# sdwyc/ROLO

Measured on AMD Instinct MI355X. Metric: scans/sec (128k-pt frame, 20 GN iters), higher is better.
Workload: dtype f64

## Files before the change

### rolo_amd/csrc/knn_cov.hip

```cpp
#include <cstdio>
#include <cstring>
#include <string.h>
#include "rolo_internal.hpp"
#include "switches.hpp"
#include "dev_math.hpp"
#include "voxel_dev.hpp"
#ifdef ROLO_KNN_ROCPRIM_SORT
#include <rocprim/rocprim.hpp>
#endif
#include <cfloat>
#include <climits>

namespace rolo {

namespace {


constexpr int BBOX_BLOCKS = 128;
constexpr int BBOX_PART = 16;

__global__ __launch_bounds__(256) void bbox_kernel(KnnPair A, int* bbox) {
  __shared__ float smn[4][3], smx[4][3];
  const int which = blockIdx.x / BBOX_BLOCKS, blk = blockIdx.x - which * BBOX_BLOCKS;
  const float4* __restrict__ p = A.c[which].xyz;
  const int n = A.c[which].n;
  float mn[3] = {FLT_MAX, FLT_MAX, FLT_MAX}, mx[3] = {-FLT_MAX, -FLT_MAX, -FLT_MAX};
  for (int i = blk * blockDim.x + threadIdx.x; i < n; i += BBOX_BLOCKS * blockDim.x) {
    float4 q = p[i];
    mn[0] = fminf(mn[0], q.x); mn[1] = fminf(mn[1], q.y); mn[2] = fminf(mn[2], q.z);
    mx[0] = fmaxf(mx[0], q.x); mx[1] = fmaxf(mx[1], q.y); mx[2] = fmaxf(mx[2], q.z);
  }
#pragma unroll
  for (int d = 0; d < 3; d++) {
#pragma unroll
    for (int off = 32; off > 0; off >>= 1) {
      mn[d] = fminf(mn[d], __shfl_xor(mn[d], off, 64));
      mx[d] = fmaxf(mx[d], __shfl_xor(mx[d], off, 64));
    }
  }
  const int wv = threadIdx.x >> 6;
  if ((threadIdx.x & 63) == 0) {
#pragma unroll
    for (int d = 0; d < 3; d++) { smn[wv][d] = mn[d]; smx[wv][d] = mx[d]; }
  }
  __syncthreads();
  if (threadIdx.x < 3) {
    const int d = threadIdx.x;
    const float a = fminf(fminf(smn[0][d], smn[1][d]), fminf(smn[2][d], smn[3][d]));
    const float b = fmaxf(fmaxf(smx[0][d], smx[1][d]), fmaxf(smx[2][d], smx[3][d]));
    int* part = bbox + BBOX_PART + (which * BBOX_BLOCKS + blk) * 6;
    part[d] = f2ord(a);
    part[3 + d] = f2ord(b);
  }
}

ROLO_DEV uint32_t expand10(uint32_t v) {
  v &= 0x3ffu;
  v = (v | (v << 16)) & 0x030000ffu;
  v = (v | (v << 8)) & 0x0300f00fu;
  v = (v | (v << 4)) & 0x030c30c3u;
  v = (v | (v << 2)) & 0x09249249u;
  return v;
}

ROLO_DEV uint32_t hilbert30(uint32_t x, uint32_t y, uint32_t z) {
  uint32_t X[3] = {x, y, z};
  for (uint32_t Q = 512; Q > 1; Q >>= 1) {
    const uint32_t P = Q - 1;
#pragma unroll
    for (int i = 0; i < 3; i++) {
      if (X[i] & Q) X[0] ^= P;
      else { const uint32_t t = (X[0] ^ X[i]) & P; X[0] ^= t; X[i] ^= t; }
    }
  }
  X[1] ^= X[0]; X[2] ^= X[1];
  uint32_t t = 0;
  for (uint32_t Q = 512; Q > 1; Q >>= 1) if (X[2] & Q) t ^= Q - 1;
  X[0] ^= t; X[1] ^= t; X[2] ^= t;
  return (expand10(X[0]) << 2) | (expand10(X[1]) << 1) | expand10(X[2]);
}

#ifndef ROLO_SORT_NB
#define ROLO_SORT_NB 128
#endif
#ifndef ROLO_SORT_T
#define ROLO_SORT_T 1024
#endif
#ifndef ROLO_SORT_EPT
#define ROLO_SORT_EPT 2
#endif
#ifndef ROLO_SORT_BITS
#define ROLO_SORT_BITS 9
#endif
#ifndef ROLO_SORT_PASSES
#define ROLO_SORT_PASSES 3
#endif
constexpr int SORT_BITS = ROLO_SORT_BITS, SORT_PASSES = ROLO_SORT_PASSES, SORT_D = 1 << SORT_BITS, KEY_BITS = SORT_BITS * SORT_PASSES;
static_assert(KEY_BITS >= 25 && KEY_BITS <= 31, "curve index + cloud bit");
constexpr int SORT_NB = ROLO_SORT_NB, SORT_T = ROLO_SORT_T;
static_assert(SORT_T % SORT_D == 0 || SORT_D % SORT_T == 0, "threads share the count prologue by digit");
static_assert(SORT_T >= 12 * 64, "the key kernel folds the 12 box components with one wavefront each");
ROLO_DEV int sort_tile(int n_total) { return ((n_total + SORT_NB - 1) / SORT_NB + SORT_T - 1) / SORT_T * SORT_T; }

constexpr int SORT_EPT = ROLO_SORT_EPT;
__global__ __launch_bounds__(SORT_T) void sort_scatter_kernel(const uint32_t* __restrict__ kin, const uint32_t* __restrict__ vin, uint32_t* __restrict__ kout,
                                                             uint32_t* __restrict__ vout, int n, int tile, int pass, int* __restrict__ cnt ,
                                                             VoxelFuse vf) {
  ROLO_ALL_KERNEL_PRIO();
  if ((int)blockIdx.x >= SORT_NB) {
    const int nt = vf.n_tgt, quarter = (nt + SORT_PASSES - 1) / SORT_PASSES;
    const int i = pass * quarter + ((int)blockIdx.x - SORT_NB) * SORT_T + (int)threadIdx.x;
    voxel_insert_point(vf.tab, vf.tgt_xyz, i < (pass + 1) * quarter ? nt : 0, i, vf.tgt_keys, vf.tgt_slot, vf.counters);
    return;
  }
  __shared__ int wcnt[SORT_T / 64][SORT_D];
  __shared__ int base[SORT_D], run[SORT_D], wsum[SORT_D / 64];
  const int tid = threadIdx.x, lane = tid & 63, wv = tid >> 6, blk = blockIdx.x;
  const int* __restrict__ c = cnt + (size_t)pass * SORT_NB * SORT_D;
  for (int k = tid; k < (SORT_T / 64) * SORT_D; k += SORT_T) (&wcnt[0][0])[k] = 0;
  constexpr int Q = SORT_T / SORT_D;
  static_assert(Q >= 1, "at least one thread per digit");
  __shared__ int part[2][Q][SORT_D];
  {
    const int d = tid & (SORT_D - 1), q = tid / SORT_D;
    int tot = 0, bef = 0;
#pragma unroll 16
    for (int b = q; b < SORT_NB; b += Q) { const int v = c[b * SORT_D + d]; tot += v; bef += b < blk ? v : 0; }
    part[0][q][d] = tot; part[1][q][d] = bef;
  }
  __syncthreads();
  int t = 0;
  if (tid < SORT_D) {
    int before = 0;
#pragma unroll
    for (int q = 0; q < Q; q++) { t += part[0][q][tid]; before += part[1][q][tid]; }
    run[tid] = before;
    int incl = t;
#pragma unroll
    for (int off = 1; off < 64; off <<= 1) { const int o = __shfl_up(incl, off, 64); if (lane >= off) incl += o; }
    if (lane == 63) wsum[wv] = incl;
    t = incl - t;
  }
  __syncthreads();
  if (tid < SORT_D) { int add = 0; for (int w = 0; w < wv; w++) add += wsum[w]; base[tid] = t + add; }
  __syncthreads();
  const int shift = SORT_BITS * pass;
  for (int r0 = 0; r0 < tile; r0 += SORT_T * SORT_EPT) {
    uint32_t key[SORT_EPT]; int off[SORT_EPT], e[SORT_EPT];
#pragma unroll
    for (int j = 0; j < SORT_EPT; j++) {
      e[j] = blk * tile + r0 + (wv * SORT_EPT + j) * 64 + lane;
      const bool valid = e[j] < n && (r0 + (wv * SORT_EPT + j) * 64 + lane) < tile;
      key[j] = valid ? kin[e[j]] : 0u;
      if (!valid) e[j] = -1;
    }
#pragma unroll
    for (int j = 0; j < SORT_EPT; j++) {
      const bool valid = e[j] >= 0;
      const int d = (int)((key[j] >> shift) & (uint32_t)(SORT_D - 1));
      unsigned long long m = __ballot(valid);
#pragma unroll
      for (int bit = 0; bit < SORT_BITS; bit++) {
        const bool one = (d >> bit) & 1;
        const unsigned long long bl = __ballot(one);
        m &= one ? bl : ~bl;
      }
      const int rank = __popcll(m & ((1ull << lane) - 1ull));
      int old = 0;
      if (valid && rank == 0) { old = wcnt[wv][d]; wcnt[wv][d] = old + __popcll(m); }
      const int leader = valid ? __ffsll((long long)m) - 1 : lane;
      old = __shfl(old, leader, 64);
      off[j] = old + rank;
    }
    __syncthreads();
    if (tid < SORT_D) {
      int acc = run[tid];
#pragma unroll
      for (int w = 0; w < SORT_T / 64; w++) { const int v = wcnt[w][tid]; wcnt[w][tid] = acc; acc += v; }
      run[tid] = acc;
    }
    __syncthreads();
#pragma unroll
    for (int j = 0; j < SORT_EPT; j++) {
      if (e[j] >= 0) {
        const int d = (int)((key[j] >> shift) & (uint32_t)(SORT_D - 1));
        const int dest = base[d] + wcnt[wv][d] + off[j];
        kout[dest] = key[j]; vout[dest] = vin[e[j]];
      }
    }
    if (r0 + SORT_T * SORT_EPT < tile) {
      __syncthreads();
      for (int k = tid; k < (SORT_T / 64) * SORT_D; k += SORT_T) (&wcnt[0][0])[k] = 0;
      __syncthreads();
    }
  }
}

constexpr int VF_CLEAR_BLOCKS = 64;
__global__ __launch_bounds__(SORT_T) void morton_kernel(KnnPair A, int* __restrict__ bbox, uint32_t* __restrict__ keys, uint32_t* __restrict__ vals, int n_total, int tile,
                                                       int* __restrict__ cnt, VoxelFuse vf) {
  ROLO_ALL_KERNEL_PRIO();
  if ((int)blockIdx.x >= SORT_NB) {
    const size_t n_words = 2 * ((size_t)vf.tab.mask + 1);
    for (size_t k = (size_t)((int)blockIdx.x - SORT_NB) * SORT_T + threadIdx.x; k < n_words; k += (size_t)VF_CLEAR_BLOCKS * SORT_T) vf.tab.keys[k] = KEY_EMPTY;
    if (blockIdx.x == SORT_NB && threadIdx.x < 3) vf.counters[threadIdx.x] = 0;
    return;
  }
  __shared__ int hist[SORT_D];
  __shared__ float par[2][4];
  const int tid = threadIdx.x, blk = blockIdx.x;
  if (tid < SORT_D) hist[tid] = 0;
  __shared__ int fin[12];
  {
    const int w = tid >> 6, lane = tid & 63;
    if (w < 6 * A.n_clouds) {
      const bool is_min = (w % 6) < 3;
      int v = is_min ? INT_MAX : INT_MIN;
      const int* __restrict__ bp = A.c[w / 6].bpart; const int nbp = A.c[w / 6].n_bpart;
      for (int b = lane; b < nbp; b += 64) { const int o = bp[b * 6 + (w % 6)]; v = is_min ? min(v, o) : max(v, o); }
#pragma unroll
      for (int off = 32; off > 0; off >>= 1) { const int o = __shfl_xor(v, off, 64); v = is_min ? min(v, o) : max(v, o); }
      if (lane == 0) { fin[w] = v; if (blk == 0) bbox[w] = v; }
    }
  }
  __syncthreads();
  if (vf.enabled && blk == 0 && tid == 0) {
    float m = 0.f;
    for (int k = 0; k < 6; k++) { const int o = fin[6 * vf.which + k]; m = fmaxf(m, fabsf(__int_as_float(o >= 0 ? o : o ^ 0x7fffffff))); }
    vf.counters[3] = __float_as_int(m);
  }
  if (tid < A.n_clouds) {
    const int* bb = fin + 6 * tid;
    const float mnx = ord2f(bb[0]), mny = ord2f(bb[1]), mnz = ord2f(bb[2]);
    const float ext = fmaxf(fmaxf(ord2f(bb[3]) - mnx, ord2f(bb[4]) - mny), ord2f(bb[5]) - mnz);
    par[tid][0] = mnx; par[tid][1] = mny; par[tid][2] = mnz; par[tid][3] = ext > 0.f ? 1024.0f / ext : 0.f;
  }
  __syncthreads();
  const int n0 = A.c[0].n;
  for (int r = tid; r < tile; r += SORT_T) {
    const int e = blk * tile + r;
    if (e >= n_total) break;
    const int which = e >= n0 ? 1 : 0;
    const int i = e - (which ? n0 : 0);
    const float4 q = A.c[which].xyz[i];
    const float mnx = par[which][0], mny = par[which][1], mnz = par[which][2], sc = par[which][3];
    const int ix = min(1023, max(0, (int)((q.x - mnx) * sc)));
    const int iy = min(1023, max(0, (int)((q.y - mny) * sc)));
    const int iz = min(1023, max(0, (int)((q.z - mnz) * sc)));
#ifndef ROLO_KNN_MORTON
    const uint32_t key = (hilbert30((uint32_t)ix, (uint32_t)iy, (uint32_t)iz) >> (31 - KEY_BITS)) | ((uint32_t)which << (KEY_BITS - 1));
#else
    const uint32_t key = ((expand10(ix) | (expand10(iy) << 1) | (expand10(iz) << 2)) >> (31 - KEY_BITS)) | ((uint32_t)which << (KEY_BITS - 1));
#endif
    keys[e] = key;
    vals[e] = (uint32_t)i;
    atomicAdd(&hist[key & (uint32_t)(SORT_D - 1)], 1);
  }
  __syncthreads();
  if (cnt && tid < SORT_D) cnt[blk * SORT_D + tid] = hist[tid];
}

__global__ __launch_bounds__(SORT_T) void sort_hist_kernel(const uint32_t* __restrict__ keys, int n, int tile, int pass, int* __restrict__ cnt) {
  ROLO_ALL_KERNEL_PRIO();
  __shared__ int hist[SORT_D];
  const int tid = threadIdx.x, blk = blockIdx.x;
  if (tid < SORT_D) hist[tid] = 0;
  __syncthreads();
  const int shift = SORT_BITS * pass;
  for (int r = tid; r < tile; r += SORT_T) {
    const int e = blk * tile + r;
    if (e >= n) break;
    atomicAdd(&hist[(keys[e] >> shift) & (uint32_t)(SORT_D - 1)], 1);
  }
  __syncthreads();
  if (tid < SORT_D) cnt[(size_t)pass * SORT_NB * SORT_D + blk * SORT_D + tid] = hist[tid];
}

__global__ __launch_bounds__(256) void leaf_kernel(KnnPair A, int split, const uint32_t* __restrict__ order) {
  ROLO_ALL_KERNEL_PRIO();
  const int which = (int)blockIdx.x >= split ? 1 : 0;
  const float4* __restrict__ p = A.c[which].xyz;
  const int n = A.c[which].n, n_leaves = A.c[which].n_leaves, P = A.c[which].P;
  float4* sorted = A.c[which].sorted; float4* boxes = A.c[which].boxes;
  order += which ? A.c[0].n : 0;
  const int s = ((int)blockIdx.x - (which ? split : 0)) * blockDim.x + threadIdx.x;
  const int g = s / KNN_LEAF;
  float4 o = make_float4(INFINITY, INFINITY, INFINITY, __int_as_float(INT_MAX));
  if (g < P && s < n) {
    const uint32_t idx = order[s];
    const float4 q = p[idx];
    o = make_float4(q.x, q.y, q.z, __int_as_float((int)idx));
  }
  if (g >= P) return;
  const bool real = __float_as_int(o.w) != INT_MAX;
  float lox = real ? o.x : INFINITY, loy = real ? o.y : INFINITY, loz = real ? o.z : INFINITY;
  float hix = real ? o.x : -INFINITY, hiy = real ? o.y : -INFINITY, hiz = real ? o.z : -INFINITY;
  if (g < n_leaves) sorted[s] = o;
#pragma unroll
  for (int m = 1; m < KNN_LEAF; m <<= 1) {
    lox = fminf(lox, __shfl_xor(lox, m)); loy = fminf(loy, __shfl_xor(loy, m)); loz = fminf(loz, __shfl_xor(loz, m));
    hix = fmaxf(hix, __shfl_xor(hix, m)); hiy = fmaxf(hiy, __shfl_xor(hiy, m)); hiz = fmaxf(hiz, __shfl_xor(hiz, m));
  }
  if ((s & (KNN_LEAF - 1)) == 0) {
    boxes[2 * (size_t)(P + g)] = make_float4(lox, loy, loz, 0.f);
    boxes[2 * (size_t)(P + g) + 1] = make_float4(hix, hiy, hiz, 0.f);
  }
  constexpr int LPB = 256 / KNN_LEAF;
  if (P >= LPB) {
    __shared__ float4 nlo[LPB], nhi[LPB];
    const int lt = threadIdx.x / KNN_LEAF;
    if ((s & (KNN_LEAF - 1)) == 0) { nlo[lt] = make_float4(lox, loy, loz, 0.f); nhi[lt] = make_float4(hix, hiy, hiz, 0.f); }
    __syncthreads();
    const size_t g0 = (size_t)P + (size_t)(g - lt);
    int m = LPB; size_t first = g0;
    while (m > 1) {
      const int half = m >> 1;
      first >>= 1;
      float4 a, b;
      const int u = threadIdx.x;
      if (u < half) {
        const float4 l0 = nlo[2 * u], l1 = nlo[2 * u + 1], h0 = nhi[2 * u], h1 = nhi[2 * u + 1];
        a = make_float4(fminf(l0.x, l1.x), fminf(l0.y, l1.y), fminf(l0.z, l1.z), 0.f);
        b = make_float4(fmaxf(h0.x, h1.x), fmaxf(h0.y, h1.y), fmaxf(h0.z, h1.z), 0.f);
      }
      __syncthreads();
      if (u < half) { nlo[u] = a; nhi[u] = b; boxes[2 * (first + u)] = a; boxes[2 * (first + u) + 1] = b; }
      __syncthreads();
      m = half;
    }
  }
}

__global__ __launch_bounds__(256) void tree_reduce_kernel(float4* boxes0, int count_in0, int chunk0, int split, float4* boxes1, int count_in1, int chunk1) {
  ROLO_ALL_KERNEL_PRIO();
  __shared__ float4 lo[512], hi[512];
  const bool second = (int)blockIdx.x >= split;
  float4* boxes = second ? boxes1 : boxes0;
  const int count_in = second ? count_in1 : count_in0, chunk = second ? chunk1 : chunk0;
  const int b = (int)blockIdx.x - (second ? split : 0), t = threadIdx.x;
  const size_t base_in = (size_t)count_in + (size_t)b * chunk;
  for (int i = t; i < chunk; i += 256) { lo[i] = boxes[2 * (base_in + i)]; hi[i] = boxes[2 * (base_in + i) + 1]; }
  __syncthreads();
  int m = chunk, level_count = count_in;
  while (m > 1) {
    const int half = m >> 1;
    level_count >>= 1;
    float4 nlo, nhi;
    if (t < half) {
      float4 a = lo[2 * t], c = lo[2 * t + 1], e = hi[2 * t], f = hi[2 * t + 1];
      nlo = make_float4(fminf(a.x, c.x), fminf(a.y, c.y), fminf(a.z, c.z), 0.f);
      nhi = make_float4(fmaxf(e.x, f.x), fmaxf(e.y, f.y), fmaxf(e.z, f.z), 0.f);
    }
    __syncthreads();
    if (t < half) {
      lo[t] = nlo; hi[t] = nhi;
      size_t h = (size_t)level_count + (size_t)b * half + t;
      boxes[2 * h] = nlo; boxes[2 * h + 1] = nhi;
    }
    __syncthreads();
    m = half;
  }
}

struct Rot2 { double c, s; };

ROLO_DEV void make_jacobi(double x, double y, double z, Rot2& r) {
  double deno = 2.0 * fabs(y);
  if (deno < DBL_MIN) { r.c = 1; r.s = 0; return; }
  double tau = (x - z) / deno;
  double w = sqrt(tau * tau + 1.0);
  double t = 1.0 / ((tau > 0) ? tau + w : tau - w);
  double n = 1.0 / sqrt(t * t + 1.0);
  const double mag = fabs(t) * n + fabs(y) * 0.0;
  const int flip = ((t > 0) ? (int)0x80000000 : 0) ^ (__double2hiint(y) & (int)0x80000000);
  r.s = __hiloint2double(__double2hiint(mag) ^ flip, __double2loint(mag));
  r.c = n;
}

template <int P_, int Q_>
ROLO_DEV bool jacobi_pair(double (&W)[9], double (&U)[9], double (&V)[9], double& max_diag) {
  const double threshold = fmax(DBL_MIN, 2.0 * DBL_EPSILON * max_diag);
  if (!(fabs(W[P_ * 3 + Q_]) > threshold || fabs(W[Q_ * 3 + P_]) > threshold)) return false;
  double m00 = W[P_ * 3 + P_], m01 = W[P_ * 3 + Q_], m10 = W[Q_ * 3 + P_], m11 = W[Q_ * 3 + Q_];
  Rot2 rot1;
  double t = m00 + m11, d = m10 - m01;
  if (fabs(d) < DBL_MIN) { rot1.s = 0; rot1.c = 1; }
  else {
    double u = t / d; double tmp = sqrt(1.0 + u * u);
    if (fabs(u) >= 0x1p-500 && tmp <= 0x1p499) { const double rt = div_den(tmp); rot1.s = div_shared(1.0, tmp, rt); rot1.c = div_shared(u, tmp, rt); }
    else { rot1.s = 1.0 / tmp; rot1.c = u / tmp; }
  }
  double n00 = rot1.c * m00 + rot1.s * m10, n01 = rot1.c * m01 + rot1.s * m11, n11 = -rot1.s * m01 + rot1.c * m11;
  Rot2 jr; make_jacobi(n00, n01, n11, jr);
  Rot2 jl; { double c2 = jr.c, s2 = -jr.s; jl.c = rot1.c * c2 - rot1.s * s2; jl.s = rot1.c * s2 + rot1.s * c2; }
#pragma unroll
  for (int k = 0; k < 3; k++) { double x = W[P_ * 3 + k], y = W[Q_ * 3 + k]; W[P_ * 3 + k] = jl.c * x + jl.s * y; W[Q_ * 3 + k] = -jl.s * x + jl.c * y; }
#pragma unroll
  for (int k = 0; k < 3; k++) { double x = U[k * 3 + P_], y = U[k * 3 + Q_]; U[k * 3 + P_] = jl.c * x + jl.s * y; U[k * 3 + Q_] = -jl.s * x + jl.c * y; }
#pragma unroll
  for (int k = 0; k < 3; k++) { double x = W[k * 3 + P_], y = W[k * 3 + Q_]; W[k * 3 + P_] = jr.c * x - jr.s * y; W[k * 3 + Q_] = jr.s * x + jr.c * y; }
#pragma unroll
  for (int k = 0; k < 3; k++) { double x = V[k * 3 + P_], y = V[k * 3 + Q_]; V[k * 3 + P_] = jr.c * x - jr.s * y; V[k * 3 + Q_] = jr.s * x + jr.c * y; }
  max_diag = fmax(max_diag, fmax(fabs(W[P_ * 3 + P_]), fabs(W[Q_ * 3 + Q_])));
  return true;
}

ROLO_DEV void swap_cols(double (&M)[9], int a, int b) {
#pragma unroll
  for (int k = 0; k < 3; k++) { double t = M[k * 3 + a]; M[k * 3 + a] = M[k * 3 + b]; M[k * 3 + b] = t; }
}

ROLO_DEV void jacobi_svd3(const double (&A)[9], double (&U)[9], double (&sv)[3], double (&V)[9]) {
  double scale = 0;
#pragma unroll
  for (int i = 0; i < 9; i++) scale = fmax(scale, fabs(A[i]));
  if (!(scale > 0) || !isfinite(scale)) scale = 1.0;
  double W[9];
#pragma unroll
  for (int i = 0; i < 9; i++) { W[i] = A[i] / scale; U[i] = (i % 4 == 0) ? 1.0 : 0.0; V[i] = (i % 4 == 0) ? 1.0 : 0.0; }
  double max_diag = fmax(fabs(W[0]), fmax(fabs(W[4]), fabs(W[8])));
  for (int sweep = 0; sweep < 100; sweep++) {
    bool any = false;
    any |= jacobi_pair<1, 0>(W, U, V, max_diag);
    any |= jacobi_pair<2, 0>(W, U, V, max_diag);
    any |= jacobi_pair<2, 1>(W, U, V, max_diag);
    if (!any) break;
  }
#pragma unroll
  for (int i = 0; i < 3; i++) {
    double a = fabs(W[i * 4]);
    sv[i] = a * scale;
    if (a != 0) { double sgn = copysign(1.0, W[i * 4]) + W[i * 4] * 0.0; U[0 * 3 + i] *= sgn; U[1 * 3 + i] *= sgn; U[2 * 3 + i] *= sgn; }
  }
  if (sv[1] > sv[0] && sv[1] >= sv[2]) { double t = sv[0]; sv[0] = sv[1]; sv[1] = t; swap_cols(U, 0, 1); swap_cols(V, 0, 1); }
  else if (sv[2] > sv[0] && sv[2] > sv[1]) { double t = sv[0]; sv[0] = sv[2]; sv[2] = t; swap_cols(U, 0, 2); swap_cols(V, 0, 2); }
  if (sv[2] > sv[1]) { double t = sv[1]; sv[1] = sv[2]; sv[2] = t; swap_cols(U, 1, 2); swap_cols(V, 1, 2); }
}

ROLO_DEV void inv3(const double (&A)[9], double (&o)[9]) {
  double c00 = A[4] * A[8] - A[5] * A[7], c01 = A[2] * A[7] - A[1] * A[8], c02 = A[1] * A[5] - A[2] * A[4];
  double c10 = A[5] * A[6] - A[3] * A[8], c11 = A[0] * A[8] - A[2] * A[6], c12 = A[2] * A[3] - A[0] * A[5];
  double c20 = A[3] * A[7] - A[4] * A[6], c21 = A[1] * A[6] - A[0] * A[7], c22 = A[0] * A[4] - A[1] * A[3];
  double det = A[0] * c00 + A[1] * c10 + A[2] * c20;
  double inv = 1.0 / det;
  o[0] = c00 * inv; o[1] = c01 * inv; o[2] = c02 * inv; o[3] = c10 * inv; o[4] = c11 * inv; o[5] = c12 * inv; o[6] = c20 * inv; o[7] = c21 * inv; o[8] = c22 * inv;
}

ROLO_DEV void knn_covariance_finish(double cxx, double cxy, double cxz, double cyy, double cyz, double czz, int n, int qi, int reg,
                                    double* __restrict__ cov, double (&c6)[6], double* __restrict__ nrm = nullptr) {
  double out[9];
  double U[9], V[9];

  if (reg == ROLO_REG_NONE) {
    out[0] = cxx; out[1] = cxy; out[2] = cxz; out[3] = cxy; out[4] = cyy; out[5] = cyz; out[6] = cxz; out[7] = cyz; out[8] = czz;
  } else if (reg == ROLO_REG_FROBENIUS) {
    double C[9] = {cxx + 1e-3, cxy, cxz, cxy, cyy + 1e-3, cyz, cxz, cyz, czz + 1e-3};
    double Ci[9]; inv3(C, Ci);
    double nrm = 0;
#pragma unroll
    for (int i = 0; i < 9; i++) nrm += Ci[i] * Ci[i];
    nrm = sqrt(nrm);
#pragma unroll
    for (int i = 0; i < 9; i++) Ci[i] /= nrm;
    inv3(Ci, out);
  } else {
    const double A[9] = {cxx, cxy, cxz, cxy, cyy, cyz, cxz, cyz, czz};
    double sv[3];
    jacobi_svd3(A, U, sv, V);
    double v0 = 1, v1 = 1, v2 = 1e-3;
    if (reg == ROLO_REG_MIN_EIG) { v0 = fmax(sv[0], 1e-3); v1 = fmax(sv[1], 1e-3); v2 = fmax(sv[2], 1e-3); }
    else if (reg == ROLO_REG_NORMALIZED_MIN_EIG) {
      const double m = fmax(sv[0], fmax(sv[1], sv[2])), q0 = sv[0] / m, q1 = sv[1] / m, q2 = sv[2] / m;
      v0 = q0 < 1e-3 ? 1e-3 : q0; v1 = q1 < 1e-3 ? 1e-3 : q1; v2 = q2 < 1e-3 ? 1e-3 : q2;
    }
    else if (reg == ROLO_REG_PLANE_S) { double s = sv[0] + sv[1] + sv[2]; v0 = sv[0] / s; v1 = sv[1] / s; v2 = 1e-3; }
#pragma unroll
    for (int a = 0; a < 3; a++)
#pragma unroll
      for (int b = 0; b < 3; b++) out[a * 3 + b] = (U[a * 3 + 0] * v0) * V[b * 3 + 0] + (U[a * 3 + 1] * v1) * V[b * 3 + 1] + (U[a * 3 + 2] * v2) * V[b * 3 + 2];
  }
  const size_t pitch = (size_t)n;
  c6[0] = out[0]; c6[1] = 0.5 * (out[1] + out[3]); c6[2] = 0.5 * (out[2] + out[6]); c6[3] = out[4]; c6[4] = 0.5 * (out[5] + out[7]); c6[5] = out[8];
  if (reg == ROLO_REG_PLANE) {
    const double s3 = U[0 * 3 + 2] * V[0 * 3 + 2] + U[1 * 3 + 2] * V[1 * 3 + 2] + U[2 * 3 + 2] * V[2 * 3 + 2];
    const double al = sqrt(1.0 - (s3 < 0 ? -1e-3 : 1e-3));
    const double mx = al * V[0 * 3 + 2], my = al * V[1 * 3 + 2], mz = al * V[2 * 3 + 2];
    const double s1 = U[0 * 3 + 0] * V[0 * 3 + 0] + U[1 * 3 + 0] * V[1 * 3 + 0] + U[2 * 3 + 0] * V[2 * 3 + 0];
    const double s2 = U[0 * 3 + 1] * V[0 * 3 + 1] + U[1 * 3 + 1] * V[1 * 3 + 1] + U[2 * 3 + 1] * V[2 * 3 + 1];
    const bool plane_form = s1 > 0 && s2 > 0;
    if (plane_form) {
      const double p6[6] = {1.0 - mx * mx, -(mx * my), -(mx * mz), 1.0 - my * my, -(my * mz), 1.0 - mz * mz};
      double dev = 0;
#pragma unroll
      for (int d = 0; d < 6; d++) dev = fmax(dev, fabs(c6[d] - p6[d]));
      if (!(dev <= 0x1p-46)) {
#pragma unroll
        for (int d = 0; d < 6; d++) c6[d] = p6[d];
      }
    }
    if (nrm) { nrm[qi] = plane_form ? mx : __builtin_nan(""); nrm[pitch + qi] = my; nrm[2 * pitch + qi] = mz; }
  }
#pragma unroll
  for (int d = 0; d < 6; d++) cov[d * pitch + qi] = c6[d];
}

template <int KMAX>
ROLO_DEV void knn_neighbourhood_moments(const int (&ki)[KMAX], int kk, const float4* __restrict__ orig, double (&m6)[6]) {
  float px[KMAX], py[KMAX], pz[KMAX];
#pragma unroll
  for (int u = 0; u < KMAX; u++) {
    const float4 p = (u < kk) ? orig[ki[u]] : make_float4(0.f, 0.f, 0.f, 0.f);
    px[u] = p.x; py[u] = p.y; pz[u] = p.z;
  }
  double mx = 0, my = 0, mz = 0;
#pragma unroll
  for (int u = 0; u < KMAX; u++) if (u < kk) { mx += (double)px[u]; my += (double)py[u]; mz += (double)pz[u]; }
  mx /= kk; my /= kk; mz /= kk;
  double cxx = 0, cxy = 0, cxz = 0, cyy = 0, cyz = 0, czz = 0;
#pragma unroll
  for (int u = 0; u < KMAX; u++) if (u < kk) {
    const double ax = (double)px[u] - mx, ay = (double)py[u] - my, az = (double)pz[u] - mz;
    cxx += ax * ax; cxy += ax * ay; cxz += ax * az; cyy += ay * ay; cyz += ay * az; czz += az * az;
  }
  m6[0] = cxx / kk; m6[1] = cxy / kk; m6[2] = cxz / kk; m6[3] = cyy / kk; m6[4] = cyz / kk; m6[5] = czz / kk;
}

template <int KMAX>
ROLO_DEV void knn_covariance_tail(const int (&ki)[KMAX], int kk, const float4* __restrict__ orig, int n, int qi, int reg,
                                  double* __restrict__ cov, double (&c6)[6], double* __restrict__ nrm = nullptr) {
  double m6[6];
  knn_neighbourhood_moments<KMAX>(ki, kk, orig, m6);
  knn_covariance_finish(m6[0], m6[1], m6[2], m6[3], m6[4], m6[5], n, qi, reg, cov, c6, nrm);
}

ROLO_DEV void knn_covariance_tail_loop(const int32_t* __restrict__ nbr, size_t n_sorted, int j, int kk, const float4* __restrict__ orig, int n, int qi, int reg,
                                       double* __restrict__ cov, double (&c6)[6], double* __restrict__ nrm = nullptr) {
  double mx = 0, my = 0, mz = 0;
  for (int u = 0; u < kk; u++) { const float4 p = orig[nbr[(size_t)u * n_sorted + j]]; mx += (double)p.x; my += (double)p.y; mz += (double)p.z; }
  mx /= kk; my /= kk; mz /= kk;
  double cxx = 0, cxy = 0, cxz = 0, cyy = 0, cyz = 0, czz = 0;
  for (int u = 0; u < kk; u++) {
    const float4 p = orig[nbr[(size_t)u * n_sorted + j]];
    const double ax = (double)p.x - mx, ay = (double)p.y - my, az = (double)p.z - mz;
    cxx += ax * ax; cxy += ax * ay; cxz += ax * az; cyy += ay * ay; cyz += ay * az; czz += az * az;
  }
  cxx /= kk; cxy /= kk; cxz /= kk; cyy /= kk; cyz /= kk; czz /= kk;
  knn_covariance_finish(cxx, cxy, cxz, cyy, cyz, czz, n, qi, reg, cov, c6, nrm);
}
}
}

#include "knn_walk.hpp"

namespace rolo {

bool knn_voxel_fuse_supported() {
#ifdef ROLO_KNN_ROCPRIM_SORT
  return false;
#else
  return true;
#endif
}

size_t knn_bbox_ints() { return BBOX_PART + 2 * BBOX_BLOCKS * 6; }

size_t knn_sort_temp_bytes(int n) {
#ifdef ROLO_KNN_ROCPRIM_SORT
  size_t bytes = 0;
  (void)rocprim::radix_sort_pairs(nullptr, bytes, (uint32_t*)nullptr, (uint32_t*)nullptr, (uint32_t*)nullptr, (uint32_t*)nullptr,
                                  (size_t)n, 0, 31, (hipStream_t)0);
  return bytes;
#else
  (void)n;
  return sizeof(int) * SORT_PASSES * SORT_NB * SORT_D;
#endif
}

hipError_t launch_knn_build(const KnnPair& A_in, void* sort_tmp, size_t sort_tmp_bytes, uint32_t* keys0, uint32_t* keys1,
                            uint32_t* vals0, uint32_t* vals1, int* bbox, const VoxelFuse& vf, hipStream_t s) {
  KnnPair A = A_in;
  bool have_parts = true;
  for (int i = 0; i < A.n_clouds; i++) have_parts = have_parts && A.c[i].bpart != nullptr && A.c[i].n_bpart > 0;
  if (!have_parts) for (int i = 0; i < A.n_clouds; i++) { A.c[i].bpart = bbox + BBOX_PART + i * BBOX_BLOCKS * 6; A.c[i].n_bpart = BBOX_BLOCKS; }
  const int nc = A.n_clouds;
  const int n_total = A.c[0].n + (nc > 1 ? A.c[1].n : 0);
#ifdef ROLO_KNN_ROCPRIM_SORT
  const int tile_ = ((n_total + SORT_NB - 1) / SORT_NB + SORT_T - 1) / SORT_T * SORT_T;
  if (!have_parts) bbox_kernel<<<BBOX_BLOCKS * nc, 256, 0, s>>>(A, bbox);
  morton_kernel<<<SORT_NB + (vf.enabled ? VF_CLEAR_BLOCKS : 0), SORT_T, 0, s>>>(A, bbox, keys0, vals0, n_total, tile_, nullptr, vf);
  hipError_t e = rocprim::radix_sort_pairs(sort_tmp, sort_tmp_bytes, keys0, keys1, vals0, vals1, (size_t)n_total, 0, nc > 1 ? KEY_BITS : KEY_BITS - 1, s);
  if (e != hipSuccess) return e;
  const uint32_t* order = vals1;
#else
  (void)sort_tmp_bytes;
  int* cnt = static_cast<int*>(sort_tmp);
  const int gvf = vf.enabled ? ((vf.n_tgt + SORT_PASSES - 1) / SORT_PASSES + SORT_T - 1) / SORT_T : 0;
  const int tile = ((n_total + SORT_NB - 1) / SORT_NB + SORT_T - 1) / SORT_T * SORT_T;
  if (!have_parts) bbox_kernel<<<BBOX_BLOCKS * nc, 256, 0, s>>>(A, bbox);
  morton_kernel<<<SORT_NB + (vf.enabled ? VF_CLEAR_BLOCKS : 0), SORT_T, 0, s>>>(A, bbox, keys0, vals0, n_total, tile, cnt, vf);
  uint32_t *ki = keys0, *vi = vals0, *ko = keys1, *vo = vals1;
  for (int p = 0; p < SORT_PASSES; p++) {
    if (p > 0) sort_hist_kernel<<<SORT_NB, SORT_T, 0, s>>>(ki, n_total, tile, p, cnt);
    sort_scatter_kernel<<<SORT_NB + gvf, SORT_T, 0, s>>>(ki, vi, ko, vo, n_total, tile, p, cnt, vf);
    uint32_t* t1 = ki; ki = ko; ko = t1; t1 = vi; vi = vo; vo = t1;
  }
  const uint32_t* order = vi;
#endif
  static_assert(256 % KNN_LEAF == 0 && (KNN_LEAF & (KNN_LEAF - 1)) == 0, "leaf_kernel reduces a leaf inside a wavefront");
  const int l0 = (A.c[0].P * KNN_LEAF + 255) / 256, l1 = nc > 1 ? (A.c[1].P * KNN_LEAF + 255) / 256 : 0;
  leaf_kernel<<<l0 + l1, 256, 0, s>>>(A, l0, order);
  constexpr int LPB = 256 / KNN_LEAF;
  int count0 = A.c[0].P >= LPB ? A.c[0].P / LPB : A.c[0].P, count1 = nc > 1 ? (A.c[1].P >= LPB ? A.c[1].P / LPB : A.c[1].P) : 1;
  while (count0 > 1 || count1 > 1) {
    const int chunk0 = count0 < 512 ? count0 : 512, chunk1 = count1 < 512 ? count1 : 512;
    const int b0 = count0 > 1 ? count0 / chunk0 : 0, b1 = count1 > 1 ? count1 / chunk1 : 0;
    tree_reduce_kernel<<<b0 + b1, 256, 0, s>>>(A.c[0].boxes, count0, chunk0, b0, nc > 1 ? A.c[1].boxes : nullptr, count1, chunk1);
    if (count0 > 1) count0 /= chunk0;
    if (count1 > 1) count1 /= chunk1;
  }
  return hipGetLastError();
}

#ifdef ROLO_KNN_STATS
extern "C" int rolo_debug_wave_records(unsigned* out ) {
  (void)hipDeviceSynchronize();
  return hipMemcpyFromSymbol(out, HIP_SYMBOL(g_knn_wave_rec), sizeof(unsigned) * 16384 * 8) == hipSuccess ? 0 : -1;
}
#endif

static inline int slice_blocks(const KnnCloud& c) { return (c.q_end - c.q_begin + 255) / 256; }

constexpr int KNN_SUB_MAX_PACKETS = 1792;
hipError_t launch_knn_walk(const KnnPair& A, int k, hipStream_t s, int* lanes_out, bool device_busy, bool moments) {
  if (lanes_out) *lanes_out = 1;
  constexpr int QPB = 256;
  const int n0 = A.c[0].q_end - A.c[0].q_begin, n1 = A.n_clouds > 1 ? A.c[1].q_end - A.c[1].q_begin : 0;
  const int g0 = (n0 + QPB - 1) / QPB, g1 = (n1 + QPB - 1) / QPB;
  if (g0 + g1 == 0) return hipSuccess;
  for (int i = 0; i < A.n_clouds; i++) if (A.c[i].q_end > A.c[i].q_begin && A.c[i].q_begin % 64 != 0) return hipErrorInvalidValue;
  for (int i = 0; i < A.n_clouds; i++) if (A.c[i].n >= KNN_MAX_POINTS) return hipErrorInvalidValue;
  if (k > 64) {
    KnnPair R = A;
    for (int r = 0; 64 * r < k; r++) {
      const int kr = k - 64 * r < 64 ? k - 64 * r : 64;
      for (int i = 0; i < R.n_clouds; i++) { R.c[i].slot0 = 64 * r; R.c[i].k_total = k; }
      if (r == 0) knn_walk_kernel<64><<<g0 + g1, 256, 0, s>>>(R, g0, kr);
      else knn_walk_kernel<64, true><<<g0 + g1, 256, 0, s>>>(R, g0, kr);
    }
    return hipGetLastError();
  }
  if (k == 20) {
    const int sub_env = switches().knn_sub;
    const int packets = (n0 + 63) / 64 + (n1 + 63) / 64;
    const int lanes = sub_env < 0 ? (packets <= KNN_SUB_MAX_PACKETS ? 4 : (device_busy ? 0 : 2)) : (sub_env == 2 ? 2 : (sub_env ? 4 : 0));
    if (lanes_out) *lanes_out = lanes ? lanes : 1;
    if (lanes == 4) { const int s0 = (n0 + 63) / 64, s1 = (n1 + 63) / 64; if (moments) knn_walk_sub_kernel<4, true><<<s0 + s1, 256, 0, s>>>(A, s0); else knn_walk_sub_kernel<4><<<s0 + s1, 256, 0, s>>>(A, s0); }
    else if (lanes == 2) { const int s0 = (n0 + 127) / 128, s1 = (n1 + 127) / 128; if (moments) knn_walk_sub_kernel<2, true><<<s0 + s1, 256, 0, s>>>(A, s0); else knn_walk_sub_kernel<2><<<s0 + s1, 256, 0, s>>>(A, s0); }
    else if (moments) knn_walk_kernel<20, false, true><<<g0 + g1, 256, 0, s>>>(A, g0, k);
    else knn_walk_kernel<20><<<g0 + g1, 256, 0, s>>>(A, g0, k);
  }
  else if (k > 32) knn_walk_kernel<64><<<g0 + g1, 256, 0, s>>>(A, g0, k);
  else knn_walk_kernel<32><<<g0 + g1, 256, 0, s>>>(A, g0, k);
  return hipGetLastError();
}

hipError_t launch_knn_unstage(const KnnPair& A, bool own_slice_only, const VoxelFuse& vf, hipStream_t s) {
  const int g0 = own_slice_only ? slice_blocks(A.c[0]) : (A.c[0].n_sorted + 255) / 256;
  const int g1 = A.n_clouds > 1 ? (own_slice_only ? slice_blocks(A.c[1]) : (A.c[1].n_sorted + 255) / 256) : 0;
  if (g0 + g1 == 0) return hipSuccess;
  VoxelFuse v = vf;
  if (own_slice_only) v.enabled = 0;
  knn_unstage_kernel<<<g0 + g1, 256, 0, s>>>(A, g0, own_slice_only ? 1 : 0, v);
  return hipGetLastError();
}

hipError_t launch_knn_tail(const KnnPair& A, int k, int regularization, const VoxelFuse& vf, hipStream_t s, bool moments) {
  const int g0 = slice_blocks(A.c[0]), g1 = A.n_clouds > 1 ? slice_blocks(A.c[1]) : 0;
  if (g0 + g1 == 0) return hipSuccess;
  if (k > 64) knn_tail_loop_kernel<<<g0 + g1, 256, 0, s>>>(A, g0, k, regularization, vf);
  else if (k == 20 && moments) knn_tail_kernel<20, true><<<g0 + g1, 256, 0, s>>>(A, g0, k, regularization, vf);
  else if (k == 20) knn_tail_kernel<20><<<g0 + g1, 256, 0, s>>>(A, g0, k, regularization, vf);
  else if (k <= 32) knn_tail_kernel<32><<<g0 + g1, 256, 0, s>>>(A, g0, k, regularization, vf);
  else knn_tail_kernel<64><<<g0 + g1, 256, 0, s>>>(A, g0, k, regularization, vf);
  return hipGetLastError();
}

}
```

Baseline: 5217.

## Sort each cloud separately in radix sort, dropping cloud bit and vals pre-write

The radix sort now gives each cloud its own half of the workgroups and its own segment of the key buffer. Keys no longer carry a cloud bit, so the curve index keeps a full 27 bits over the three passes. The key kernel stops writing a vals array, because the first scatter pass derives the value from the element index. The per-digit count prologue only sums rows for the block's own cloud, in unrolled chunks. It also removes the rocprim path. The changes trim memory traffic and prologue work but add per-block geometry arithmetic.

```diff
diff --git a/rolo_amd/csrc/knn_cov.hip b/rolo_amd/csrc/knn_cov.hip
--- a/rolo_amd/csrc/knn_cov.hip
+++ b/rolo_amd/csrc/knn_cov.hip
@@ -5,9 +5,7 @@
 #include "switches.hpp"
 #include "dev_math.hpp"
 #include "voxel_dev.hpp"
-#ifdef ROLO_KNN_ROCPRIM_SORT
-#include <rocprim/rocprim.hpp>
-#endif
+#include "sort_tiles.hpp"
 #include <cfloat>
 #include <climits>
 
@@ -80,12 +78,6 @@
   return (expand10(X[0]) << 2) | (expand10(X[1]) << 1) | expand10(X[2]);
 }
 
-#ifndef ROLO_SORT_NB
-#define ROLO_SORT_NB 128
-#endif
-#ifndef ROLO_SORT_T
-#define ROLO_SORT_T 1024
-#endif
 #ifndef ROLO_SORT_EPT
 #define ROLO_SORT_EPT 2
 #endif
@@ -96,16 +88,14 @@
 #define ROLO_SORT_PASSES 3
 #endif
 constexpr int SORT_BITS = ROLO_SORT_BITS, SORT_PASSES = ROLO_SORT_PASSES, SORT_D = 1 << SORT_BITS, KEY_BITS = SORT_BITS * SORT_PASSES;
-static_assert(KEY_BITS >= 25 && KEY_BITS <= 31, "curve index + cloud bit");
-constexpr int SORT_NB = ROLO_SORT_NB, SORT_T = ROLO_SORT_T;
-static_assert(SORT_T % SORT_D == 0 || SORT_D % SORT_T == 0, "threads share the count prologue by digit");
-static_assert(SORT_T >= 12 * 64, "the key kernel folds the 12 box components with one wavefront each");
-ROLO_DEV int sort_tile(int n_total) { return ((n_total + SORT_NB - 1) / SORT_NB + SORT_T - 1) / SORT_T * SORT_T; }
+static_assert(KEY_BITS >= 1 && KEY_BITS <= 30, "the leading bits of the 30-bit curve index");
+static_assert(SORT_T % SORT_D == 0, "threads share the count prologue by digit");
+static_assert(SORT_T >= 6 * 64, "the key kernel folds the 6 box components of its cloud with one wavefront each");
 
 constexpr int SORT_EPT = ROLO_SORT_EPT;
 __global__ __launch_bounds__(SORT_T) void sort_scatter_kernel(const uint32_t* __restrict__ kin, const uint32_t* __restrict__ vin, uint32_t* __restrict__ kout,
-                                                             uint32_t* __restrict__ vout, int n, int tile, int pass, int* __restrict__ cnt ,
-                                                             VoxelFuse vf) {
+                                                             uint32_t* __restrict__ vout, int n0, int n1, int n_clouds, int pass,
+                                                             int* __restrict__ cnt , VoxelFuse vf) {
   ROLO_ALL_KERNEL_PRIO();
   if ((int)blockIdx.x >= SORT_NB) {
     const int nt = vf.n_tgt, quarter = (nt + SORT_PASSES - 1) / SORT_PASSES;
@@ -115,18 +105,34 @@
   }
   __shared__ int wcnt[SORT_T / 64][SORT_D];
   __shared__ int base[SORT_D], run[SORT_D], wsum[SORT_D / 64];
-  const int tid = threadIdx.x, lane = tid & 63, wv = tid >> 6, blk = blockIdx.x;
-  const int* __restrict__ c = cnt + (size_t)pass * SORT_NB * SORT_D;
+  const int tid = threadIdx.x, lane = tid & 63, wv = tid >> 6;
+  const SortGeom g = sort_geom((int)blockIdx.x, n0, n1, n_clouds);
+  const int* __restrict__ c = cnt + ((size_t)pass * SORT_NB + g.row0) * SORT_D;
   for (int k = tid; k < (SORT_T / 64) * SORT_D; k += SORT_T) (&wcnt[0][0])[k] = 0;
-  constexpr int Q = SORT_T / SORT_D;
+  constexpr int Q = SORT_T / SORT_D, CH = 16;
   static_assert(Q >= 1, "at least one thread per digit");
+  static_assert((SORT_NB / 2) % (Q * CH) == 0, "whole chunks of rows per thread, for a pair's cloud and for a lone one");
   __shared__ int part[2][Q][SORT_D];
   {
     const int d = tid & (SORT_D - 1), q = tid / SORT_D;
-    int tot = 0, bef = 0;
-#pragma unroll 16
-    for (int b = q; b < SORT_NB; b += Q) { const int v = c[b * SORT_D + d]; tot += v; bef += b < blk ? v : 0; }
-    part[0][q][d] = tot; part[1][q][d] = bef;
+    const int nbef = g.tile > q ? (g.tile - q + Q - 1) / Q : 0;
+    int bef = 0, aft = 0;
+    for (int i0 = 0; i0 < g.tiles / Q; i0 += CH) {
+      int v[CH];
+#pragma unroll
+      for (int i = 0; i < CH; i++) v[i] = c[(q + (i0 + i) * Q) * SORT_D + d];
+      if (i0 + CH <= nbef) {
+#pragma unroll
+        for (int i = 0; i < CH; i++) bef += v[i];
+      } else if (i0 >= nbef) {
+#pragma unroll
+        for (int i = 0; i < CH; i++) aft += v[i];
+      } else {
+#pragma unroll
+        for (int i = 0; i < CH; i++) { if (i0 + i < nbef) bef += v[i]; else aft += v[i]; }
+      }
+    }
+    part[0][q][d] = bef + aft; part[1][q][d] = bef;
   }
   __syncthreads();
   int t = 0;
@@ -145,12 +151,14 @@
   if (tid < SORT_D) { int add = 0; for (int w = 0; w < wv; w++) add += wsum[w]; base[tid] = t + add; }
   __syncthreads();
   const int shift = SORT_BITS * pass;
-  for (int r0 = 0; r0 < tile; r0 += SORT_T * SORT_EPT) {
+  kin += g.offset; kout += g.offset; vout += g.offset;
+  if (pass > 0) vin += g.offset;
+  for (int r0 = 0; r0 < g.len; r0 += SORT_T * SORT_EPT) {
     uint32_t key[SORT_EPT]; int off[SORT_EPT], e[SORT_EPT];
 #pragma unroll
     for (int j = 0; j < SORT_EPT; j++) {
-      e[j] = blk * tile + r0 + (wv * SORT_EPT + j) * 64 + lane;
-      const bool valid = e[j] < n && (r0 + (wv * SORT_EPT + j) * 64 + lane) < tile;
+      e[j] = g.first + r0 + (wv * SORT_EPT + j) * 64 + lane;
+      const bool valid = e[j] < g.last;
       key[j] = valid ? kin[e[j]] : 0u;
       if (!valid) e[j] = -1;
     }
@@ -185,10 +193,10 @@
       if (e[j] >= 0) {
         const int d = (int)((key[j] >> shift) & (uint32_t)(SORT_D - 1));
         const int dest = base[d] + wcnt[wv][d] + off[j];
-        kout[dest] = key[j]; vout[dest] = vin[e[j]];
+        kout[dest] = key[j]; vout[dest] = pass > 0 ? vin[e[j]] : (uint32_t)e[j];
       }
     }
-    if (r0 + SORT_T * SORT_EPT < tile) {
+    if (r0 + SORT_T * SORT_EPT < g.len) {
       __syncthreads();
       for (int k = tid; k < (SORT_T / 64) * SORT_D; k += SORT_T) (&wcnt[0][0])[k] = 0;
       __syncthreads();
@@ -197,8 +205,7 @@
 }
 
 constexpr int VF_CLEAR_BLOCKS = 64;
-__global__ __launch_bounds__(SORT_T) void morton_kernel(KnnPair A, int* __restrict__ bbox, uint32_t* __restrict__ keys, uint32_t* __restrict__ vals, int n_total, int tile,
-                                                       int* __restrict__ cnt, VoxelFuse vf) {
+__global__ __launch_bounds__(SORT_T) void morton_kernel(KnnPair A, int* __restrict__ bbox, uint32_t* __restrict__ keys, int* __restrict__ cnt, VoxelFuse vf) {
   ROLO_ALL_KERNEL_PRIO();
   if ((int)blockIdx.x >= SORT_NB) {
     const size_t n_words = 2 * ((size_t)vf.tab.mask + 1);
@@ -207,71 +214,66 @@
     return;
   }
   __shared__ int hist[SORT_D];
-  __shared__ float par[2][4];
+  __shared__ float par[4];
   const int tid = threadIdx.x, blk = blockIdx.x;
+  const SortGeom g = sort_geom(blk, A.c[0].n, A.c[1].n, A.n_clouds);
+  const KnnCloud& C = A.c[g.cloud];
   if (tid < SORT_D) hist[tid] = 0;
-  __shared__ int fin[12];
+  __shared__ int fin[6];
   {
     const int w = tid >> 6, lane = tid & 63;
-    if (w < 6 * A.n_clouds) {
-      const bool is_min = (w % 6) < 3;
+    if (w < 6) {
+      const bool is_min = w < 3;
       int v = is_min ? INT_MAX : INT_MIN;
-      const int* __restrict__ bp = A.c[w / 6].bpart; const int nbp = A.c[w / 6].n_bpart;
-      for (int b = lane; b < nbp; b += 64) { const int o = bp[b * 6 + (w % 6)]; v = is_min ? min(v, o) : max(v, o); }
+      const int* __restrict__ bp = C.bpart; const int nbp = C.n_bpart;
+      for (int b = lane; b < nbp; b += 64) { const int o = bp[b * 6 + w]; v = is_min ? min(v, o) : max(v, o); }
 #pragma unroll
       for (int off = 32; off > 0; off >>= 1) { const int o = __shfl_xor(v, off, 64); v = is_min ? min(v, o) : max(v, o); }
-      if (lane == 0) { fin[w] = v; if (blk == 0) bbox[w] = v; }
-    }
-  }
-  __syncthreads();
-  if (vf.enabled && blk == 0 && tid == 0) {
+      if (lane == 0) { fin[w] = v; if (g.tile == 0) bbox[6 * g.cloud + w] = v; }
+    }
+  }
+  __syncthreads();
+  if (vf.enabled && g.cloud == vf.which && g.tile == 0 && tid == 0) {
     float m = 0.f;
-    for (int k = 0; k < 6; k++) { const int o = fin[6 * vf.which + k]; m = fmaxf(m, fabsf(__int_as_float(o >= 0 ? o : o ^ 0x7fffffff))); }
+    for (int k = 0; k < 6; k++) { const int o = fin[k]; m = fmaxf(m, fabsf(__int_as_float(o >= 0 ? o : o ^ 0x7fffffff))); }
     vf.counters[3] = __float_as_int(m);
   }
-  if (tid < A.n_clouds) {
-    const int* bb = fin + 6 * tid;
-    const float mnx = ord2f(bb[0]), mny = ord2f(bb[1]), mnz = ord2f(bb[2]);
-    const float ext = fmaxf(fmaxf(ord2f(bb[3]) - mnx, ord2f(bb[4]) - mny), ord2f(bb[5]) - mnz);
-    par[tid][0] = mnx; par[tid][1] = mny; par[tid][2] = mnz; par[tid][3] = ext > 0.f ? 1024.0f / ext : 0.f;
-  }
-  __syncthreads();
-  const int n0 = A.c[0].n;
-  for (int r = tid; r < tile; r += SORT_T) {
-    const int e = blk * tile + r;
-    if (e >= n_total) break;
-    const int which = e >= n0 ? 1 : 0;
-    const int i = e - (which ? n0 : 0);
-    const float4 q = A.c[which].xyz[i];
-    const float mnx = par[which][0], mny = par[which][1], mnz = par[which][2], sc = par[which][3];
+  if (tid == 0) {
+    const float mnx = ord2f(fin[0]), mny = ord2f(fin[1]), mnz = ord2f(fin[2]);
+    const float ext = fmaxf(fmaxf(ord2f(fin[3]) - mnx, ord2f(fin[4]) - mny), ord2f(fin[5]) - mnz);
+    par[0] = mnx; par[1] = mny; par[2] = mnz; par[3] = ext > 0.f ? 1024.0f / ext : 0.f;
+  }
+  __syncthreads();
+  const float4* __restrict__ xyz = C.xyz;
+  keys += g.offset;
+  const float mnx = par[0], mny = par[1], mnz = par[2], sc = par[3];
+  for (int i = g.first + tid; i < g.last; i += SORT_T) {
+    const float4 q = xyz[i];
     const int ix = min(1023, max(0, (int)((q.x - mnx) * sc)));
     const int iy = min(1023, max(0, (int)((q.y - mny) * sc)));
     const int iz = min(1023, max(0, (int)((q.z - mnz) * sc)));
 #ifndef ROLO_KNN_MORTON
-    const uint32_t key = (hilbert30((uint32_t)ix, (uint32_t)iy, (uint32_t)iz) >> (31 - KEY_BITS)) | ((uint32_t)which << (KEY_BITS - 1));
+    const uint32_t key = hilbert30((uint32_t)ix, (uint32_t)iy, (uint32_t)iz) >> (30 - KEY_BITS);
 #else
-    const uint32_t key = ((expand10(ix) | (expand10(iy) << 1) | (expand10(iz) << 2)) >> (31 - KEY_BITS)) | ((uint32_t)which << (KEY_BITS - 1));
+    const uint32_t key = (expand10(ix) | (expand10(iy) << 1) | (expand10(iz) << 2)) >> (30 - KEY_BITS);
 #endif
-    keys[e] = key;
-    vals[e] = (uint32_t)i;
+    keys[i] = key;
     atomicAdd(&hist[key & (uint32_t)(SORT_D - 1)], 1);
   }
   __syncthreads();
-  if (cnt && tid < SORT_D) cnt[blk * SORT_D + tid] = hist[tid];
-}
-
-__global__ __launch_bounds__(SORT_T) void sort_hist_kernel(const uint32_t* __restrict__ keys, int n, int tile, int pass, int* __restrict__ cnt) {
+  if (tid < SORT_D) cnt[blk * SORT_D + tid] = hist[tid];
+}
+
+__global__ __launch_bounds__(SORT_T) void sort_hist_kernel(const uint32_t* __restrict__ keys, int n0, int n1, int n_clouds, int pass, int* __restrict__ cnt) {
   ROLO_ALL_KERNEL_PRIO();
   __shared__ int hist[SORT_D];
   const int tid = threadIdx.x, blk = blockIdx.x;
+  const SortGeom g = sort_geom(blk, n0, n1, n_clouds);
   if (tid < SORT_D) hist[tid] = 0;
   __syncthreads();
   const int shift = SORT_BITS * pass;
-  for (int r = tid; r < tile; r += SORT_T) {
-    const int e = blk * tile + r;
-    if (e >= n) break;
-    atomicAdd(&hist[(keys[e] >> shift) & (uint32_t)(SORT_D - 1)], 1);
-  }
+  keys += g.offset;
+  for (int i = g.first + tid; i < g.last; i += SORT_T) atomicAdd(&hist[(keys[i] >> shift) & (uint32_t)(SORT_D - 1)], 1);
   __syncthreads();
   if (tid < SORT_D) cnt[(size_t)pass * SORT_NB * SORT_D + blk * SORT_D + tid] = hist[tid];
 }
@@ -554,26 +556,13 @@
 
 namespace rolo {
 
-bool knn_voxel_fuse_supported() {
-#ifdef ROLO_KNN_ROCPRIM_SORT
-  return false;
-#else
-  return true;
-#endif
-}
+bool knn_voxel_fuse_supported() { return true; }
 
 size_t knn_bbox_ints() { return BBOX_PART + 2 * BBOX_BLOCKS * 6; }
 
 size_t knn_sort_temp_bytes(int n) {
-#ifdef ROLO_KNN_ROCPRIM_SORT
-  size_t bytes = 0;
-  (void)rocprim::radix_sort_pairs(nullptr, bytes, (uint32_t*)nullptr, (uint32_t*)nullptr, (uint32_t*)nullptr, (uint32_t*)nullptr,
-                                  (size_t)n, 0, 31, (hipStream_t)0);
-  return bytes;
-#else
   (void)n;
   return sizeof(int) * SORT_PASSES * SORT_NB * SORT_D;
-#endif
 }
 
 hipError_t launch_knn_build(const KnnPair& A_in, void* sort_tmp, size_t sort_tmp_bytes, uint32_t* keys0, uint32_t* keys1,
@@ -583,29 +572,20 @@
   for (int i = 0; i < A.n_clouds; i++) have_parts = have_parts && A.c[i].bpart != nullptr && A.c[i].n_bpart > 0;
   if (!have_parts) for (int i = 0; i < A.n_clouds; i++) { A.c[i].bpart = bbox + BBOX_PART + i * BBOX_BLOCKS * 6; A.c[i].n_bpart = BBOX_BLOCKS; }
   const int nc = A.n_clouds;
-  const int n_total = A.c[0].n + (nc > 1 ? A.c[1].n : 0);
-#ifdef ROLO_KNN_ROCPRIM_SORT
-  const int tile_ = ((n_total + SORT_NB - 1) / SORT_NB + SORT_T - 1) / SORT_T * SORT_T;
-  if (!have_parts) bbox_kernel<<<BBOX_BLOCKS * nc, 256, 0, s>>>(A, bbox);
-  morton_kernel<<<SORT_NB + (vf.enabled ? VF_CLEAR_BLOCKS : 0), SORT_T, 0, s>>>(A, bbox, keys0, vals0, n_total, tile_, nullptr, vf);
-  hipError_t e = rocprim::radix_sort_pairs(sort_tmp, sort_tmp_bytes, keys0, keys1, vals0, vals1, (size_t)n_total, 0, nc > 1 ? KEY_BITS : KEY_BITS - 1, s);
-  if (e != hipSuccess) return e;
-  const uint32_t* order = vals1;
-#else
-  (void)sort_tmp_bytes;
+  if (nc < 2) A.c[1].n = 0;
+  const int n0 = A.c[0].n, n1 = A.c[1].n;
+  if (sort_tmp_bytes < knn_sort_temp_bytes(n0 + n1)) return hipErrorInvalidValue;
   int* cnt = static_cast<int*>(sort_tmp);
   const int gvf = vf.enabled ? ((vf.n_tgt + SORT_PASSES - 1) / SORT_PASSES + SORT_T - 1) / SORT_T : 0;
-  const int tile = ((n_total + SORT_NB - 1) / SORT_NB + SORT_T - 1) / SORT_T * SORT_T;
   if (!have_parts) bbox_kernel<<<BBOX_BLOCKS * nc, 256, 0, s>>>(A, bbox);
-  morton_kernel<<<SORT_NB + (vf.enabled ? VF_CLEAR_BLOCKS : 0), SORT_T, 0, s>>>(A, bbox, keys0, vals0, n_total, tile, cnt, vf);
+  morton_kernel<<<SORT_NB + (vf.enabled ? VF_CLEAR_BLOCKS : 0), SORT_T, 0, s>>>(A, bbox, keys0, cnt, vf);
   uint32_t *ki = keys0, *vi = vals0, *ko = keys1, *vo = vals1;
   for (int p = 0; p < SORT_PASSES; p++) {
-    if (p > 0) sort_hist_kernel<<<SORT_NB, SORT_T, 0, s>>>(ki, n_total, tile, p, cnt);
-    sort_scatter_kernel<<<SORT_NB + gvf, SORT_T, 0, s>>>(ki, vi, ko, vo, n_total, tile, p, cnt, vf);
+    if (p > 0) sort_hist_kernel<<<SORT_NB, SORT_T, 0, s>>>(ki, n0, n1, nc, p, cnt);
+    sort_scatter_kernel<<<SORT_NB + gvf, SORT_T, 0, s>>>(ki, vi, ko, vo, n0, n1, nc, p, cnt, vf);
     uint32_t* t1 = ki; ki = ko; ko = t1; t1 = vi; vi = vo; vo = t1;
   }
   const uint32_t* order = vi;
-#endif
   static_assert(256 % KNN_LEAF == 0 && (KNN_LEAF & (KNN_LEAF - 1)) == 0, "leaf_kernel reduces a leaf inside a wavefront");
   const int l0 = (A.c[0].P * KNN_LEAF + 255) / 256, l1 = nc > 1 ? (A.c[1].P * KNN_LEAF + 255) / 256 : 0;
   leaf_kernel<<<l0 + l1, 256, 0, s>>>(A, l0, order);
diff --git a/rolo_amd/csrc/sort_tiles.hpp b/rolo_amd/csrc/sort_tiles.hpp
--- /dev/null
+++ b/rolo_amd/csrc/sort_tiles.hpp
@@ -0,0 +1,54 @@
+#pragma once
+
+#if defined(__HIPCC__) || defined(__CUDACC__)
+#define ROLO_SORT_FN __host__ __device__ __forceinline__
+#else
+#define ROLO_SORT_FN inline
+#endif
+
+#ifndef ROLO_SORT_NB
+#define ROLO_SORT_NB 128
+#endif
+#ifndef ROLO_SORT_T
+#define ROLO_SORT_T 1024
+#endif
+
+namespace rolo {
+
+constexpr int SORT_NB = ROLO_SORT_NB;
+constexpr int SORT_T = ROLO_SORT_T;
+static_assert(SORT_NB >= 2 && SORT_NB % 2 == 0, "a pair gives each cloud half of the workgroups");
+
+struct SortGeom {
+  int cloud;
+  int tile;
+  int tiles;
+  int row0;
+  int len;
+  int first;
+  int last;
+  int offset;
+};
+
+ROLO_SORT_FN int sort_tile_len(int n_c, bool pair) {
+  const int per = pair ? (n_c + SORT_NB / 2 - 1) / (SORT_NB / 2) : (n_c + SORT_NB - 1) / SORT_NB;
+  return (per + SORT_T - 1) / SORT_T * SORT_T;
+}
+
+ROLO_SORT_FN SortGeom sort_geom(int blk, int n0, int n1, int n_clouds) {
+  SortGeom g;
+  const bool pair = n_clouds > 1;
+  g.tiles = pair ? SORT_NB / 2 : SORT_NB;
+  g.cloud = pair && blk >= SORT_NB / 2 ? 1 : 0;
+  g.row0 = g.cloud ? SORT_NB / 2 : 0;
+  g.tile = blk - g.row0;
+  const int n_c = g.cloud ? n1 : n0;
+  g.len = sort_tile_len(n_c, pair);
+  const int lo = g.tile * g.len;
+  g.first = lo < n_c ? lo : n_c;
+  g.last = n_c - g.first < g.len ? n_c : g.first + g.len;
+  g.offset = g.cloud ? n0 : 0;
+  return g;
+}
+
+}
```

Result: no change. 5250, median of 6 (+0.6%).
